# ImIntheMiddle/VATL4Pose-WACV2024

Measured on AMD Instinct MI355X. Metric: frames/sec pose-infer+uncertainty, 256x192 17-kp, higher is better.
Workload: dtype f32; 1 GPU; SimpleBaseline-R50 256x192 inference + decode + local-peak + THC-L1, 1024-frame synthetic video per GPU; frames_per_gpu=1024, batch=1024, tracks=4, parallelism=frame-sharded x1

## Files before the change

### include/vatl_hip.h

```cpp
#ifndef VATL_HIP_H
#define VATL_HIP_H

#include <stdint.h>

#ifdef __cplusplus
extern "C" {
#endif

#define VATL_VERSION 100
#define VATL_EINVAL  (-1)
#define VATL_ELAUNCH (-2)

int         vatl_version(void);
const char* vatl_last_error(void);

int vatl_flop_meter_begin(void);
int vatl_flop_meter_end(double* direct_flops, double* winograd_flops, int64_t* direct_launches, int64_t* winograd_launches);
#define VATL_ROUTE_NAMES "igemm,igemm_bnbwd,igemm_dma,persistent_1x1,streamk,rows_1x1,bottleneck_chain,stem_pool,halo_3x3," \
                         "winograd,winograd_2h,winograd_bnbwd,winograd_persist,winograd_c32,wgrad,winograd_wgrad,winograd_wgrad_2h," \
                         "winograd_wgrad_table,winograd_f4,winograd_f4_bnbwd,gemm1x1_ring"
int vatl_flop_meter_routes(int64_t* counts, int n);


int vatl_nchw_to_nhwc(const float* src, float* dst, int N, int C, int H, int W, int Cpad, void* stream);
int vatl_nhwc_to_nchw(const float* src, float* dst, int N, int C, int H, int W, void* stream);

int vatl_pack_conv_weight(const float* w_oihw, float* w_packed, int Cout, int Cin, int R, int S,
                          int CoutPad, int Spad, int CinPad, void* stream);
int vatl_pack_deconv4x4s2_weight(const float* w_iohw, float* w_packed, int Cin, int Cout, int CoutPad, void* stream);
int64_t vatl_stem_pool_weight_floats(void);
int vatl_pack_stem_pool_weight(const float* w_oihw, float* packed, void* stream);
int vatl_stem_pool_supported(int H, int W);
int vatl_stem7x7s2_pool_fwd(const float* x_nchw, const float* w_packed, const float* scale, const float* bias, float* y_nhwc,
                            int N, int H, int W, void* stream);
int64_t vatl_stem3_weight_floats(void);
int vatl_pack_stem3_weight(const float* w_oihw, float* packed, void* stream);
int vatl_stem3x3s2_fwd(const float* x_nchw, const float* w_packed, const float* scale, const float* bias, float* y_nhwc,
                       int N, int H, int W, void* stream);

int vatl_bn_fold(const float* gamma, const float* beta, const float* mean, const float* var, const float* conv_bias,
                 float eps, float* scale, float* bias, int C, void* stream);


// ... 209 lines not shown
                     int32_t* indices_dev, int32_t* tie_flag_dev, double* workspace, void* stream);
int vatl_kmeans_assign(const double* xc, const double* centers, int64_t n, int D, int k, const int32_t* labels_prev_or_null, int32_t* labels,
                       double* status, double* workspace, void* stream);
int64_t vatl_kmeans_update_workspace_doubles(int D, int k);
int vatl_kmeans_update(const double* xc, const double* weight, const int32_t* labels, const double* centers, int64_t n, int D, int k,
                       double* centers_new, double* status, double* workspace, void* stream);
int vatl_kmeans_finish(const float* emb, const double* xc, const double* mean, const double* weight, const double* centers,
                       const int32_t* labels, int64_t n, int D, int k, int32_t* representatives, double* inertia, double* workspace,
                       void* stream);

int vatl_winograd_cout_pad(int Cout);
int64_t vatl_winograd_weight_floats(int Cout, int Cin);
int vatl_pack_winograd_weight(const float* w, float* u, int Cout, int Cin, int data_gradient, void* stream);
int vatl_conv3x3_winograd_fwd(const float* x, const float* u, const float* scale, const float* bias, const float* residual, float* y,
                              int N, int H, int W, int Cin, int Cout, int relu, void* stream);
int vatl_winograd_last_route(void);
int64_t vatl_winograd_stats_row_blocks(int64_t N, int H, int W);
int vatl_conv3x3_winograd_fwd_stats(const float* x, const float* u, float* y, double* stats, int64_t* row_blocks_used, int N, int H, int W,
                                    int Cin, int Cout, void* stream);
int64_t vatl_winograd_deconv_weight_floats(int Cout, int Cin);
int vatl_pack_winograd_deconv_weight(const float* w, float* u, int Cout, int Cin, void* stream);
int vatl_deconv4x4s2_winograd_fwd(const float* x, const float* u, const float* scale, const float* bias, float* y, int N, int H, int W,
                                  int Cin, int Cout, int relu, void* stream);
int64_t vatl_winograd_deconv_stats_row_blocks(int64_t N, int H, int W);
int vatl_deconv4x4s2_winograd_fwd_stats(const float* x, const float* u, float* y, double* stats, int64_t* row_blocks_used, int N, int H, int W,
                                        int Cin, int Cout, void* stream);
int64_t vatl_conv3x3_winograd_wgrad_workspace_floats(int Cout, int Cin, int64_t N, int H, int W);
int vatl_conv3x3_winograd_wgrad(const float* x, const float* dz, float* dw, float* workspace, int N, int H, int W, int Cin, int Cout, void* stream);
int64_t vatl_deconv4x4s2_winograd_wgrad_workspace_floats(int Cin, int Cout, int64_t N, int H, int W);
int vatl_deconv4x4s2_winograd_wgrad(const float* x, const float* dy, float* dw, float* workspace, int N, int H, int W, int Cin, int Cout,
                                    void* stream);
int64_t vatl_winograd_deconv_dgrad_weight_floats(int Cin, int Cout);
int vatl_pack_winograd_deconv_dgrad_weight(const float* w, float* u, int Cin, int Cout, void* stream);
int vatl_deconv4x4s2_winograd_dgrad(const float* dz, const float* u, const float* residual, float* dx, int N, int H, int W, int Cin, int Cout,
                                    void* stream);
int vatl_deconv4x4s2_winograd_dgrad_bnbwd(const float* dz, const float* u, const float* residual, float* dx, int N, int H, int W, int Cin,
                                          int Cout, const float* bn_z, const float* bn_mask_y, const float* bn_scale, const float* bn_bias,
                                          const float* bn_mean, const float* bn_invstd, double* stats, int64_t* row_blocks_used, void* stream);
int vatl_conv3x3_winograd_fwd_bnbwd(const float* x, const float* u, const float* residual, float* y, int N, int H, int W, int Cin, int Cout,
                                    const float* bn_z, const float* bn_mask_y, const float* bn_scale, const float* bn_bias,
                                    const float* bn_mean, const float* bn_invstd, double* stats, int64_t* row_blocks_used, void* stream);

int64_t vatl_checksum_block_words(void);
int vatl_checksum_multi(const int64_t* table_dev, int n_tensors, int64_t total_blocks, uint64_t* out, void* stream);

#ifdef __cplusplus
// ... 4 lines not shown
```

### vatl4pose-wacv2024_amd/alphapose/models/hip_engine.py

```python
from __future__ import annotations

import time
import weakref

import torch
import torch.nn as nn

import vatl_hip as vh

MAX_CHUNK = 1024



WINOGRAD = True
ROWS_GEMM = True
ROWS_GEMM_K = (128, 256)
WINO_C32 = True
WINO_F4 = True


class _Conv:
    __slots__ = ("w", "u", "u32", "u4", "wsrc", "wino", "c32", "f4", "scale", "bias", "cout", "r", "s", "stride", "pad")

    def __init__(self, conv: nn.Conv2d, bn: nn.BatchNorm2d | None):
        assert conv.groups == 1 and conv.dilation == (1, 1)
        assert conv.stride[0] == conv.stride[1] and conv.padding[0] == conv.padding[1]
        self.w = vh.pack_conv_weight(conv.weight.detach())
        self.cout, _, self.r, self.s = conv.weight.shape
        self.stride, self.pad = conv.stride[0], conv.padding[0]
        self.u = self.u32 = self.u4 = None
        self.wino = WINOGRAD and (self.r, self.s, self.stride, self.pad) == (3, 3, 1, 1) and conv.in_channels % 16 == 0 and self.cout % 4 == 0
        self.c32 = self.wino and WINO_C32 and conv.in_channels == 32 and self.cout == 32
        self.f4 = self.wino and WINO_F4 and conv.in_channels >= 64 and conv.in_channels % 16 == 0 and self.cout % 64 == 0
        self.wsrc = conv.weight.detach() if self.wino else None
        cb = conv.bias.detach() if conv.bias is not None else None
        if bn is not None:
            self.scale, self.bias = vh.bn_fold(_d(bn.weight), _d(bn.bias), bn.running_mean, bn.running_var, bn.eps, cb)
        elif cb is not None:
            self.scale, self.bias = vh.bn_fold(None, None, None, None, 0.0, cb, channels=self.cout)
        else:
            self.scale = self.bias = None

    def __call__(self, x, relu, residual=None, out_nchw=False, out=None):
        if self.wino and not out_nchw and not vh.latency_mode():
            if self.c32 and vh.conv3x3_winograd_c32_supported(x.shape[0], x.shape[1], x.shape[2], 32, 32):
                if self.u32 is None:
                    self.u32 = vh.pack_winograd_c32_weight(self.wsrc)
                return vh.conv3x3_winograd_c32_fwd(x, self.u32, self.scale, self.bias, relu, residual=residual, out=out)
            if self.f4 and vh.conv3x3_winograd_f4_supported(x.shape[0], x.shape[1], x.shape[2], x.shape[3], self.cout):
                if self.u4 is None:
                    self.u4 = vh.pack_winograd_f4_weight(self.wsrc)
                return vh.conv3x3_winograd_f4_fwd(x, self.u4, self.scale, self.bias, self.cout, relu, residual=residual, out=out)
            if self.u is None:
                self.u = vh.pack_winograd_weight(self.wsrc)
            return vh.conv3x3_winograd_fwd(x, self.u, self.scale, self.bias, self.cout, relu, residual=residual, out=out)
        if (ROWS_GEMM and self.r == 1 and self.stride == 1 and not out_nchw and not vh.latency_mode() and x.shape[-1] in ROWS_GEMM_K
                and vh.conv1x1_rows_supported(x.shape[-1], 0, self.cout, x.shape[0] * x.shape[1] * x.shape[2])):
            return vh.conv1x1_rows_fwd(x, self.w, self.scale, self.bias, self.cout, relu, residual=residual, out=out)
        return vh.conv2d_fwd(x, self.w, self.scale, self.bias, self.cout, self.r, self.s, self.stride, self.pad, relu,
                             residual=residual, out_nchw=out_nchw, out=out)


class _Deconv:
    __slots__ = ("w", "u", "scale", "bias", "cout")

    def __init__(self, dc: nn.ConvTranspose2d, bn: nn.BatchNorm2d):
        assert dc.kernel_size == (4, 4) and dc.stride == (2, 2) and dc.padding == (1, 1) and dc.bias is None
        self.cout = dc.weight.shape[1]
        self.u = None
        if WINOGRAD and dc.weight.shape[0] % 16 == 0 and self.cout % 4 == 0:
            self.u = vh.pack_winograd_deconv_weight(dc.weight.detach())
        self.w = vh.pack_deconv_weight(dc.weight.detach())
        self.scale, self.bias = vh.bn_fold(_d(bn.weight), _d(bn.bias), bn.running_mean, bn.running_var, bn.eps)

    def __call__(self, x, relu=True):
        if self.u is not None and not vh.latency_mode():
            return vh.deconv4x4s2_winograd_fwd(x, self.u, self.scale, self.bias, self.cout, relu)
        return vh.deconv4x4s2_fwd(x, self.w, self.scale, self.bias, self.cout, relu)


def _d(p):
    return None if p is None else p.detach()


FUSE_PROJ = True


class _BottleneckPlan:
    def __init__(self, blk):
        self.c1 = _Conv(blk.conv1, blk.bn1)
        self.c2 = _Conv(blk.conv2, blk.bn2)
        self.c3 = _Conv(blk.conv3, blk.bn3)
        self.proj = _Conv(blk.downsample[0], blk.downsample[1]) if blk.downsample is not None else None
        self.dual = None
        if (FUSE_PROJ and self.proj is not None and type(self) is _BottleneckPlan and self.proj.r == 1 and self.c3.cout >= 128
                and blk.conv3.in_channels % 32 == 0 and blk.downsample[0].in_channels % 32 == 0):
            w, b = vh.pack_conv1x1_dual_weight(blk.conv3.weight.detach(), self.c3.scale, self.c3.bias, blk.downsample[0].weight.detach(),
                                               self.proj.scale, self.proj.bias)
            self.dual = (w, b, self.proj.stride)

# ... 469 lines not shown
```

### vatl4pose-wacv2024_amd/csrc/common.h

```cpp
#pragma once
#include <hip/hip_runtime.h>
#include <atomic>
#include <cstdarg>
#include <cstdio>
#include <cstdint>

#include "vatl_hip.h"

namespace vatl {

char* err_buf();
int fail(int code, const char* fmt, ...);

void meter_add(int kind, double flops);
enum MeterRoute {
    kRouteIgemm = 0, kRouteIgemmBnBwd, kRouteIgemmDma, kRoutePersistent1x1, kRouteStreamK, kRouteRows, kRouteChain, kRouteStemPool, kRouteHalo,
    kRouteWino, kRouteWino2H, kRouteWinoBnBwd, kRouteWinoPersist, kRouteWinoC32, kRouteWgrad, kRouteWinoWgrad, kRouteWinoWgrad2H,
    kRouteWinoWgradTable, kRouteWinoF4, kRouteWinoF4BnBwd, kRouteGemm1x1Ring, kRouteCount
};
void meter_route(int route);

inline int check_launch(const char* what) {
    hipError_t e = hipGetLastError();
    if (e != hipSuccess) return fail(VATL_ELAUNCH, "%s: %s", what, hipGetErrorString(e));
    return 0;
}

inline int ensure_dynamic_lds(const void* kern, int bytes, std::atomic<unsigned>& done_mask, const char* what) {
    int d = 0;
    if (hipGetDevice(&d) != hipSuccess) return fail(VATL_ELAUNCH, "%s: no current device", what);
    const unsigned bit = 1u << (d & 31);
    if (done_mask.load(std::memory_order_acquire) & bit) return 0;
    hipError_t e = hipFuncSetAttribute(kern, hipFuncAttributeMaxDynamicSharedMemorySize, bytes);
    if (e != hipSuccess) return fail(VATL_ELAUNCH, "hipFuncSetAttribute(%s): %s", what, hipGetErrorString(e));
    done_mask.fetch_or(bit, std::memory_order_release);
    return 0;
}

__attribute__((visibility("hidden"))) int conv3x3_halo_try(const float* x, const float* w, const float* scale, const float* bias, const float* residual, float* y, int N, int H, int W,
                                                           int Cin, int Cout, int CoutPad, int R, int S, int stride, int pad, int relu, hipStream_t st);

// ... 51 lines not shown
```

### vatl4pose-wacv2024_amd/csrc/pack.hip

```cpp
#include "glue_common.h"
#include "winograd_pack.h"

namespace vatl {

template <class I>
__device__ __forceinline__ float pack_conv_elem(const float* __restrict__ w, I i, int Cout, int Cin, int R, int S, int Spad, int CinPad) {
    const I c = i % (I)CinPad;
    I t = i / (I)CinPad;
    const I s = t % (I)Spad; t /= (I)Spad;
    const I r = t % (I)R;
    const I o = t / (I)R;
    float v = 0.f;
    if ((int)o < Cout && (int)s < S && (int)c < Cin) v = w[(((long long)o * Cin + c) * R + r) * S + s];
    return v;
}

template <class I>
__device__ __forceinline__ float pack_deconv_elem(const float* __restrict__ w, I i, int Cin, int Cout, int CoutPad) {
    const I c = i % (I)Cin;
    I t = i / (I)Cin;
    const int tx = (int)(t & 1); t >>= 1;
    const int ty = (int)(t & 1); t >>= 1;
    const I o = t % (I)CoutPad;
    const int ph = (int)(t / (I)CoutPad);
// ... 54 lines not shown
    for (long long i = blockIdx.x * (long long)blockDim.x + threadIdx.x; i < total; i += (long long)gridDim.x * blockDim.x) {
        const int k = (int)(i % K), o = (int)(i / K);
        float v = 0.f;
        if (o < Cout) v = k < C1 ? w1[(long long)o * C1 + k] * s1[o] : w2[(long long)o * C2 + (k - C1)] * s2[o];
        out[i] = v;
        if (k == 0 && o < Cout) bias[o] = b1[o] + b2[o];
    }
}

__global__ void bn_fold_kernel(const float* gamma, const float* beta, const float* mean, const float* var, const float* cbias,
                               float eps, float* scale, float* bias, int C) {
    const int c = blockIdx.x * blockDim.x + threadIdx.x;
    if (c >= C) return;
    float s = 1.f, b = 0.f;
    if (var) {
        s = (gamma ? gamma[c] : 1.f) / sqrtf(var[c] + eps);
        b = (beta ? beta[c] : 0.f) - mean[c] * s;
    }
    if (cbias) b += cbias[c] * s;
    scale[c] = s;
    bias[c] = b;
}

__global__ __launch_bounds__(256) void pack_multi_kernel(const VatlPackJob* __restrict__ jobs, int njobs) {
    __shared__ int sj;
    if (threadIdx.x == 0) {
        int lo = 0, hi = njobs - 1;
        const long long b = blockIdx.x;
        while (lo < hi) {
            const int mid = (lo + hi + 1) >> 1;
            if (jobs[mid].first_block <= b) lo = mid; else hi = mid - 1;
        }
        sj = lo;
    }
    __syncthreads();
    const VatlPackJob* J = jobs + sj;
    const float* __restrict__ w = J->src;
    float* __restrict__ out = J->dst;
    const int kind = J->kind, Cout = J->Cout, Cin = J->Cin, R = J->R, S = J->S, pa = J->a, pb = J->b, pc = J->c;
    if (kind >= 7) {
        f4_pack_item(w, out, kind - 7, pc, Cout, Cin, ((long long)blockIdx.x - J->first_block) * 256 + threadIdx.x);
        return;
    }
    if (kind >= 3) {
        wino_pack_block(w, out, kind - 3, pc, Cout, Cin, pb, (long long)blockIdx.x - J->first_block, threadIdx.x);
        return;
// ... 20 lines not shown
using namespace vatl;

extern "C" int vatl_pack_conv_weight(const float* w, float* out, int Cout, int Cin, int R, int S, int CoutPad, int Spad, int CinPad, void* stream) {
    if (!w || !out || CoutPad < Cout || Spad < S || CinPad < Cin) return fail(VATL_EINVAL, "pack_conv_weight: bad arguments");
    hipLaunchKernelGGL(pack_conv_weight_kernel, dim3(ew_grid((long long)CoutPad * R * Spad * CinPad)), dim3(256), 0, (hipStream_t)stream,
                       w, out, Cout, Cin, R, S, CoutPad, Spad, CinPad);
    return check_launch("pack_conv_weight");
}

extern "C" int vatl_pack_conv1x1_dual_weight(const float* w1, const float* scale1, const float* bias1, const float* w2, const float* scale2,
                                             const float* bias2, float* out, float* bias, int Cout, int C1, int C2, int CoutPad, void* stream) {
    if (!w1 || !scale1 || !bias1 || !w2 || !scale2 || !bias2 || !out || !bias || CoutPad < Cout) return fail(VATL_EINVAL, "pack_conv1x1_dual_weight: bad arguments");
    hipLaunchKernelGGL(pack_dual_weight_kernel, dim3(ew_grid((long long)CoutPad * (C1 + C2))), dim3(256), 0, (hipStream_t)stream, w1, scale1, bias1, w2,
                       scale2, bias2, out, bias, Cout, C1, C2, CoutPad);
    return check_launch("pack_conv1x1_dual_weight");
}

extern "C" int vatl_pack_deconv4x4s2_weight(const float* w, float* out, int Cin, int Cout, int CoutPad, void* stream) {
    if (!w || !out || CoutPad < Cout) return fail(VATL_EINVAL, "pack_deconv4x4s2_weight: bad arguments");
    hipLaunchKernelGGL(pack_deconv_weight_kernel, dim3(ew_grid(16LL * CoutPad * Cin)), dim3(256), 0, (hipStream_t)stream, w, out, Cin, Cout, CoutPad);
    return check_launch("pack_deconv4x4s2_weight");
}

extern "C" int vatl_pack_dgrad_weight(const float* w_oihw, float* out, int Cout, int Cin, int R, int S, int CinPad, int CoutK,
                                      int ntaps, const int* tap_r, const int* tap_s, void* stream) {
    if (!w_oihw || !out || !tap_r || !tap_s || ntaps < 1 || ntaps > 16 || CinPad < Cin || CoutK < Cout) return fail(VATL_EINVAL, "pack_dgrad_weight: bad arguments");
    TapList t{};
    t.n = ntaps;
    for (int i = 0; i < ntaps; ++i) {
        if (tap_r[i] < 0 || tap_r[i] >= R || tap_s[i] < 0 || tap_s[i] >= S) return fail(VATL_EINVAL, "pack_dgrad_weight: tap %d out of range", i);
        t.r[i] = tap_r[i]; t.s[i] = tap_s[i];
    }
    hipLaunchKernelGGL(pack_dgrad_weight_kernel, dim3((unsigned)((long long)cdiv(CinPad, 32) * ntaps * cdiv(CoutK, 32))), dim3(256), 0, (hipStream_t)stream,
                       w_oihw, out, Cout, Cin, R, S, CinPad, CoutK, t);
    return check_launch("pack_dgrad_weight");
}

extern "C" int vatl_pack_weights_multi(const VatlPackJob* jobs_device, int njobs, int64_t total_blocks, void* stream) {
    if (njobs == 0) return 0;
    if (!jobs_device || njobs < 0 || total_blocks <= 0 || total_blocks > 0x7FFFFFFF) return fail(VATL_EINVAL, "pack_weights_multi: bad arguments");
    hipLaunchKernelGGL(pack_multi_kernel, dim3((unsigned)total_blocks), dim3(256), 0, (hipStream_t)stream, jobs_device, njobs);
    return check_launch("pack_weights_multi");
}

extern "C" int vatl_bn_fold(const float* gamma, const float* beta, const float* mean, const float* var, const float* conv_bias,
                            float eps, float* scale, float* bias, int C, void* stream) {
// ... 5 lines not shown
```

### vatl4pose-wacv2024_amd/csrc/winograd_pack.h

```cpp
#pragma once

namespace vatl {

__device__ __forceinline__ void wino_pack_block(const float* __restrict__ w, float* __restrict__ out, int mode, int w_i, int Cout, int Cin, int NH,
                                                long long bl, int tid) {
    const int steps = Cin >> 3;
    int phase = 0;
    if (mode >= 2) {
        const long long per = (long long)((Cout + 32 * NH - 1) / (32 * NH)) * NH * steps;
        phase = (int)(bl / per);
        bl -= phase * per;
        out += phase * per * 4096;
    }
    const int n32 = (int)(bl / steps), step = (int)(bl - (long long)n32 * steps);
    const int nl = tid & 31, cc = tid >> 5;
    const int n = n32 * 32 + nl, c = step * 8 + cc;
    const int n_tile = n32 / NH, nh = n32 - n_tile * NH;
    const int lane = (cc >> 2) * 32 + nl, tt = cc & 3;
    double tg[4][3];
    if (mode >= 2) {
        const int py = phase >> 1, px = phase & 1;
        double g[2][2];
#pragma unroll
        for (int a = 0; a < 2; ++a)
// ... 20 lines not shown
                double v = 0.0;
                if (n < Cout) v = mode == 0 ? (double)w[((long long)n * w_i + c) * 9 + r * 3 + s] : (double)w[((long long)c * w_i + n) * 9 + (2 - r) * 3 + (2 - s)];
                g[r][s] = v;
            }
#pragma unroll
        for (int s = 0; s < 3; ++s) {
            tg[0][s] = g[0][s];
            tg[1][s] = 0.5 * (g[0][s] + g[1][s] + g[2][s]);
            tg[2][s] = 0.5 * (g[0][s] - g[1][s] + g[2][s]);
            tg[3][s] = g[2][s];
        }
    }
    float* o = out + ((((long long)(n_tile * steps + step) * 16) * NH + nh) * 64 + lane) * 4 + tt;
#pragma unroll
    for (int a = 0; a < 4; ++a) {
        double uu[4];
        if (mode >= 2) { uu[0] = tg[a][0]; uu[1] = 0.5 * (tg[a][0] + tg[a][1]); uu[2] = 0.5 * (tg[a][0] - tg[a][1]); uu[3] = -tg[a][1]; }
        else { uu[0] = tg[a][0]; uu[1] = 0.5 * (tg[a][0] + tg[a][1] + tg[a][2]); uu[2] = 0.5 * (tg[a][0] - tg[a][1] + tg[a][2]); uu[3] = tg[a][2]; }
#pragma unroll
        for (int b = 0; b < 4; ++b) o[(long long)(a * 4 + b) * NH * 256] = (float)uu[b];
    }
}

__device__ __forceinline__ void f4_pack_item(const float* __restrict__ w, float* __restrict__ u, int dgrad, int w_i, int Cout, int Cin, long long id) {
    const int nbg = Cout >> 4;
    const long long total = (long long)(Cin >> 4) * 36 * nbg * 64;
    if (id >= total) return;
    const int lane = (int)(id & 63);
    const int blk = (int)((id >> 6) % nbg);
    const int pos = (int)((id >> 6) / nbg % 36);
    const int stage = (int)((id >> 6) / nbg / 36);
    const int xi = pos / 6, nu = pos - 6 * xi;
    const double G[6][3] = {{0.25, 0, 0}, {-1.0 / 6, -1.0 / 6, -1.0 / 6}, {-1.0 / 6, 1.0 / 6, -1.0 / 6}, {1.0 / 24, 1.0 / 12, 1.0 / 6}, {1.0 / 24, -1.0 / 12, 1.0 / 6}, {0, 0, 1}};
    const int n = 16 * blk + (lane & 15);
    float o[4];
#pragma unroll
    for (int s = 0; s < 4; ++s) {
        const int c = 16 * stage + 4 * (lane >> 4) + s;
        const float* g = dgrad ? w + ((long long)c * w_i + n) * 9 : w + ((long long)n * w_i + c) * 9;
        double v = 0.0;
#pragma unroll
        for (int i = 0; i < 3; ++i)
#pragma unroll
            for (int j = 0; j < 3; ++j) v += G[xi][i] * (double)(dgrad ? g[(2 - i) * 3 + (2 - j)] : g[i * 3 + j]) * G[nu][j];
        o[s] = (float)v;
    }
// ... 6 lines not shown
```

### vatl4pose-wacv2024_amd/vatl_hip/__init__.py

```python
from __future__ import annotations

import ctypes as C
import os
import threading as _threading

import torch

_HERE = os.path.dirname(os.path.abspath(__file__))
LIB_PATH = os.environ.get("VATL_HIP_LIB") or os.path.join(_HERE, "libvatl_hip.so")

_p = C.c_void_p
_i = C.c_int
_f = C.c_float
_d = C.c_double
_i64 = C.c_int64

SIGNATURES = {
    "vatl_version": (_i, []),
    "vatl_last_error": (C.c_char_p, []),
    "vatl_flop_meter_begin": (_i, []),
    "vatl_flop_meter_end": (_i, [_p, _p, _p, _p]),
    "vatl_flop_meter_routes": (_i, [_p, _i]),
    "vatl_nchw_to_nhwc": (_i, [_p, _p, _i, _i, _i, _i, _i, _p]),
    "vatl_nhwc_to_nchw": (_i, [_p, _p, _i, _i, _i, _i, _p]),
# ... 65 lines not shown
    "vatl_scale_bias_act": (_i, [_p, _p, _p, _p, _p, _i64, _i, _i, _p]),
    "vatl_bn_train_bwd": (_i, [_p, _p, _p, _p, _p, _p, _p, _p, _p, _p, _i64, _i, _p, _p, _p]),
    "vatl_bn_train_bwd_relu": (_i, [_p, _p, _p, _p, _p, _p, _p, _p, _p, _p, _i64, _i, _p, _p, _p]),
    "vatl_conv_stats_row_blocks": (_i64, [_i64, _i]),
    "vatl_winograd_cout_pad": (_i, [_i]),
    "vatl_winograd_weight_floats": (_i64, [_i, _i]),
    "vatl_pack_winograd_weight": (_i, [_p, _p, _i, _i, _i, _p]),
    "vatl_conv3x3_winograd_fwd": (_i, [_p] * 6 + [_i] * 6 + [_p]),
    "vatl_winograd_last_route": (_i, []),
    "vatl_winograd_stats_row_blocks": (_i64, [_i64, _i, _i]),
    "vatl_conv3x3_winograd_fwd_stats": (_i, [_p, _p, _p, _p, _p, _i, _i, _i, _i, _i, _p]),
    "vatl_conv3x3_winograd_fwd_bnbwd": (_i, [_p] * 4 + [_i] * 5 + [_p] * 9),
    "vatl_conv3x3_winograd_wgrad_workspace_floats": (_i64, [_i, _i, _i64, _i, _i]),
    "vatl_conv3x3_winograd_wgrad": (_i, [_p] * 4 + [_i] * 5 + [_p]),
    "vatl_deconv4x4s2_winograd_wgrad_workspace_floats": (_i64, [_i, _i, _i64, _i, _i]),
    "vatl_deconv4x4s2_winograd_wgrad": (_i, [_p] * 4 + [_i] * 5 + [_p]),
    "vatl_winograd_deconv_dgrad_weight_floats": (_i64, [_i, _i]),
    "vatl_pack_winograd_deconv_dgrad_weight": (_i, [_p, _p, _i, _i, _p]),
    "vatl_deconv4x4s2_winograd_dgrad": (_i, [_p] * 4 + [_i] * 5 + [_p]),
    "vatl_deconv4x4s2_winograd_dgrad_bnbwd": (_i, [_p] * 4 + [_i] * 5 + [_p] * 9),
    "vatl_winograd_deconv_weight_floats": (_i64, [_i, _i]),
    "vatl_pack_winograd_deconv_weight": (_i, [_p, _p, _i, _i, _p]),
    "vatl_deconv4x4s2_winograd_fwd": (_i, [_p] * 5 + [_i] * 6 + [_p]),
    "vatl_winograd_deconv_stats_row_blocks": (_i64, [_i64, _i, _i]),
    "vatl_deconv4x4s2_winograd_fwd_stats": (_i, [_p, _p, _p, _p, _p, _i, _i, _i, _i, _i, _p]),
    "vatl_conv2d_fwd_stats": (_i, [_p, _p, _p, _p, _p, _i, _i, _i, _i, _i, _i, _i, _i, _i, _i, _p]),
    "vatl_deconv4x4s2_fwd_stats": (_i, [_p, _p, _p, _p, _p, _i, _i, _i, _i, _i, _i, _p]),
    "vatl_bn_train_finalize": (_i, [_p, _i64, _i64, _i, _p, _p, _p, _p, _f, _f, _p, _p, _p, _p, _p]),
    "vatl_maxpool3x3s2_bwd": (_i, [_p, _p, _p, _i, _i, _i, _i, _p]),
    "vatl_maxpool3x3s2_fwd_idx": (_i, [_p, _p, _p, _i, _i, _i, _i, _p]),
    "vatl_pack_weights_multi": (_i, [_p, _i, _i64, _p]),
    "vatl_adamw_multi_block_elems": (_i64, []),
    "vatl_checksum_block_words": (_i64, []),
    "vatl_checksum_multi": (_i, [_p, _i, _i64, _p, _p]),
    "vatl_maxpool3x3s2_fwd_idx_affine": (_i, [_p, _p, _p, _p, _p, _i, _i, _i, _i, _p]),
    "vatl_bn_train_bwd_relu_pool": (_i, [_p, _p, _p, _p, _p, _p, _p, _p, _p, _p, _p, _i, _i, _i, _i, _p, _p, _p]),
    "vatl_maxpool3x3s2_bwd_idx": (_i, [_p, _p, _p, _i, _i, _i, _i, _p]),
    "vatl_pixelunshuffle2": (_i, [_p, _p, _i, _i, _i, _i, _p]),
    "vatl_se_bwd": (_i, [_p, _p, _p, _p, _p, _p, _p, _p, _i, _i, _i, _p]),
    "vatl_relu_bwd": (_i, [_p, _p, _p, _i64, _p]),
    "vatl_col_sum": (_i, [_p, _i64, _i, _p, _p, _p]),
    "vatl_masked_mse_workspace_floats": (_i64, [_i64]),
    "vatl_masked_mse_fwd_bwd": (_i, [_p, _p, _p, _p, _p, _p, _i, _i, _i, _p]),
    "vatl_l1_joint_regression_fwd_bwd": (_i, [_p, _p, _p, _p, _p, _p, _p, _i, _i, _i, _i, _i, _i, _p]),
    "vatl_gaussian_targets": (_i, [_p, _p, _p, _p, _i, _i, _i, _i, _i, _i, _f, _p]),
    "vatl_crop_warp_affine": (_i, [_p, _p, _p, _p, _p, _p, _i, _i, _i, _f, _f, _f, _p]),
# ... 82 lines not shown

_tls = _threading.local()



def nchw_to_nhwc(x: torch.Tensor, cpad: int | None = None) -> torch.Tensor:
    n, c, h, w = x.shape
    cpad = cpad or c
    y = torch.empty((n, h, w, cpad), device=x.device, dtype=torch.float32)
    _check(lib().vatl_nchw_to_nhwc(_ptr(x), _ptr(y), n, c, h, w, cpad, _stream()), "vatl_nchw_to_nhwc")
    return y


def nhwc_to_nchw(x: torch.Tensor) -> torch.Tensor:
    n, h, w, c = x.shape
    y = torch.empty((n, c, h, w), device=x.device, dtype=torch.float32)
    _check(lib().vatl_nhwc_to_nchw(_ptr(x), _ptr(y), n, c, h, w, _stream()), "vatl_nhwc_to_nchw")
    return y



ROUTE_NAMES = ("igemm", "igemm_bnbwd", "igemm_dma", "persistent_1x1", "streamk", "rows_1x1", "bottleneck_chain", "stem_pool", "halo_3x3", "winograd",
               "winograd_2h", "winograd_bnbwd", "winograd_persist", "winograd_c32", "wgrad", "winograd_wgrad", "winograd_wgrad_2h", "winograd_wgrad_table", "winograd_f4", "winograd_f4_bnbwd",
               "gemm1x1_ring")


class flop_meter:

    def __enter__(self):
        _check(lib().vatl_flop_meter_begin(), "flop_meter_begin")
        self.direct = self.winograd = self.total = 0.0
        self.direct_launches = self.winograd_launches = 0
        return self

    @staticmethod
    def launches_now() -> int:
        counts = (C.c_int64 * len(ROUTE_NAMES))()
        _check(min(0, lib().vatl_flop_meter_routes(counts, len(ROUTE_NAMES))), "flop_meter_routes")
        return int(sum(counts))

    def __exit__(self, *exc):
        counts = (C.c_int64 * len(ROUTE_NAMES))()
        _check(min(0, lib().vatl_flop_meter_routes(counts, len(ROUTE_NAMES))), "flop_meter_routes")
        self.routes = {n: int(c) for n, c in zip(ROUTE_NAMES, counts)}
        d, w, nd, nw = C.c_double(0), C.c_double(0), C.c_int64(0), C.c_int64(0)
        _check(lib().vatl_flop_meter_end(C.byref(d), C.byref(w), C.byref(nd), C.byref(nw)), "flop_meter_end")
        self.direct, self.winograd, self.total = d.value, w.value, d.value + w.value
# ... 240 lines not shown
    cout, cin = (ci, co) if data_gradient else (co, ci)
    return _pack(("winograd", w.data_ptr(), tuple(w.shape), bool(data_gradient)), w, lambda: (
        int(lib().vatl_winograd_weight_floats(cout, cin)), "vatl_pack_winograd_weight", (cout, cin, int(data_gradient)),
        _winograd_fields(_PACK_WINOGRAD_DGRAD if data_gradient else _PACK_WINOGRAD, cout, cin, 3, ci)))


def pack_winograd_f4_weight(w: torch.Tensor, data_gradient: bool = False) -> torch.Tensor:
    co, ci = w.shape[:2]
    cout, cin = (ci, co) if data_gradient else (co, ci)
    return _pack(("winograd_f4", w.data_ptr(), tuple(w.shape), bool(data_gradient)), w, lambda: (
        int(lib().vatl_winograd_f4_weight_floats(cout, cin)), "vatl_pack_winograd_f4_weight", (cout, cin, int(data_gradient)),
        (_PACK_WINOGRAD_F4_DGRAD if data_gradient else _PACK_WINOGRAD_F4, cout, cin, 3, 3, 0, 0, ci, ())))


def pack_winograd_deconv_weight(w: torch.Tensor) -> torch.Tensor:
    cin, cout = w.shape[:2]
    if tuple(w.shape[2:]) != (4, 4):
        raise VatlError("pack_winograd_deconv_weight: 4x4 filters only")
    return _pack(("winograd_deconv", w.data_ptr(), tuple(w.shape)), w, lambda: (
        int(lib().vatl_winograd_deconv_weight_floats(cout, cin)), "vatl_pack_winograd_deconv_weight", (cout, cin),
        _winograd_fields(_PACK_WINOGRAD_DECONV, cout, cin, 4, cout)))


def pack_winograd_deconv_dgrad_weight(w: torch.Tensor) -> torch.Tensor:
    cin, cout = w.shape[:2]
    if tuple(w.shape[2:]) != (4, 4):
        raise VatlError("pack_winograd_deconv_dgrad_weight: 4x4 filters only")
    return _pack(("winograd_deconv_dgrad", w.data_ptr(), tuple(w.shape)), w, lambda: (
        int(lib().vatl_winograd_deconv_dgrad_weight_floats(cin, cout)), "vatl_pack_winograd_deconv_dgrad_weight", (cin, cout),
        _winograd_fields(_PACK_WINOGRAD_DECONV_DGRAD, cin, cout, 4, cout)))


def pack_conv1x1_dual_weight(w1, scale1, bias1, w2, scale2, bias2):
    cout, c1 = w1.shape[:2]
    c2 = w2.shape[1]
    cpad = conv_cout_pad(cout)
    out = torch.empty((cpad, c1 + c2), device=w1.device, dtype=torch.float32)
    bias = torch.empty(cout, device=w1.device, dtype=torch.float32)
    _check(lib().vatl_pack_conv1x1_dual_weight(_ptr(w1.contiguous()), _ptr(scale1), _ptr(bias1), _ptr(w2.contiguous()), _ptr(scale2), _ptr(bias2),
                                               _ptr(out), _ptr(bias), cout, c1, c2, cpad, _stream()), "vatl_pack_conv1x1_dual_weight")
    return out, bias


def pack_winograd_c32_weight(w: torch.Tensor) -> torch.Tensor:
    if tuple(w.shape) != (32, 32, 3, 3):
        raise VatlError("pack_winograd_c32_weight: a (32, 32, 3, 3) filter")
# ... 126 lines not shown
    return y


def conv3x3_winograd_f4_supported(n: int, h: int, w: int, cin: int, cout: int) -> bool:
    return bool(lib().vatl_conv3x3_winograd_f4_supported(n, h, w, cin, cout))


def conv3x3_winograd_f4_fwd(x, u, scale, bias, cout: int, relu: bool, residual=None, out=None):
    n, h, w, cin = x.shape
    y = out if out is not None else torch.empty((n, h, w, cout), device=x.device, dtype=torch.float32)
    _check(lib().vatl_conv3x3_winograd_f4_fwd(_ptr(x), _ptr(u), _ptr(scale), _ptr(bias), _ptr(residual), _ptr(y), n, h, w, cin, cout, int(relu), _stream()),
           "vatl_conv3x3_winograd_f4_fwd")
    return y


def deconv4x4s2_fwd(x, w_packed, scale, bias, cout: int, relu: bool):
    n, h, w, cin = x.shape
    y = torch.empty((n, 2 * h, 2 * w, cout), device=x.device, dtype=torch.float32)
    _check(lib().vatl_deconv4x4s2_fwd(_ptr(x), _ptr(w_packed), _ptr(scale), _ptr(bias), _ptr(y), n, h, w, cin, cout,
                                      w_packed.shape[1], int(relu), _stream()), "vatl_deconv4x4s2_fwd")
    return y


def deconv4x4s2_winograd_fwd(x, u_packed, scale, bias, cout: int, relu: bool, out=None):
    n, h, w, cin = x.shape
    y = out if out is not None else torch.empty((n, 2 * h, 2 * w, cout), device=x.device, dtype=torch.float32)
    _check(lib().vatl_deconv4x4s2_winograd_fwd(_ptr(x), _ptr(u_packed), _ptr(scale), _ptr(bias), _ptr(y), n, h, w, cin, cout, int(relu), _stream()),
           "vatl_deconv4x4s2_winograd_fwd")
    return y


def maxpool3x3s2_fwd(x):
    n, h, w, c = x.shape
    y = torch.empty((n, (h - 1) // 2 + 1, (w - 1) // 2 + 1, c), device=x.device, dtype=torch.float32)
    _check(lib().vatl_maxpool3x3s2_fwd(_ptr(x), _ptr(y), n, h, w, c, _stream()), "vatl_maxpool3x3s2_fwd")
    return y


def gap_fwd(x):
    n, h, w, c = x.shape
    y = torch.empty((n, c), device=x.device, dtype=torch.float32)
    _check(lib().vatl_gap_fwd(_ptr(x), _ptr(y), n, h * w, c, _stream()), "vatl_gap_fwd")
    return y


def pixelshuffle2_fwd(x):
    n, h, w, c = x.shape
    y = torch.empty((n, 2 * h, 2 * w, c // 4), device=x.device, dtype=torch.float32)
    _check(lib().vatl_pixelshuffle2_fwd(_ptr(x), _ptr(y), n, h, w, c, _stream()), "vatl_pixelshuffle2_fwd")
# ... 751 lines not shown
```

Before: 16340 frames/s.

## Add F(4x3,2x2) Winograd kernel for stride-2 deconvolution phases

Adds a new Winograd kernel for the 4x4 stride-2 deconvolution. Each of the four output phases is treated as a 2x2 conv and computed with larger output tiles: 4 rows by 3 columns and 20 transform points. The kernel uses MFMA 32x32x2 f32, buffer loads straight into LDS, double-buffered stages and XCD-aware block remapping. The aim is fewer multiplies per output and better reuse than the existing deconv Winograd path. The packed weights are built lazily on the first supported call. The trade-offs are extra numerical error from the larger transform, an extra packed-weight buffer, and shape restrictions (H%4, W%3, Cout%64).

```diff
diff --git a/include/vatl_hip.h b/include/vatl_hip.h
--- a/include/vatl_hip.h
+++ b/include/vatl_hip.h
@@ -18,7 +18,7 @@
 int vatl_flop_meter_end(double* direct_flops, double* winograd_flops, int64_t* direct_launches, int64_t* winograd_launches);
 #define VATL_ROUTE_NAMES "igemm,igemm_bnbwd,igemm_dma,persistent_1x1,streamk,rows_1x1,bottleneck_chain,stem_pool,halo_3x3," \
                          "winograd,winograd_2h,winograd_bnbwd,winograd_persist,winograd_c32,wgrad,winograd_wgrad,winograd_wgrad_2h," \
-                         "winograd_wgrad_table,winograd_f4,winograd_f4_bnbwd,gemm1x1_ring"
+                         "winograd_wgrad_table,winograd_f4,winograd_f4_bnbwd,gemm1x1_ring,winograd_deconv43"
 int vatl_flop_meter_routes(int64_t* counts, int n);
 
 
@@ -274,6 +274,11 @@
 int vatl_pack_winograd_deconv_weight(const float* w, float* u, int Cout, int Cin, void* stream);
 int vatl_deconv4x4s2_winograd_fwd(const float* x, const float* u, const float* scale, const float* bias, float* y, int N, int H, int W,
                                   int Cin, int Cout, int relu, void* stream);
+int64_t vatl_winograd_deconv43_weight_floats(int Cout, int Cin);
+int vatl_pack_winograd_deconv43_weight(const float* w, float* u, int Cout, int Cin, void* stream);
+int vatl_deconv4x4s2_winograd43_supported(int N, int H, int W, int Cin, int Cout);
+int vatl_deconv4x4s2_winograd43_fwd(const float* x, const float* u, const float* scale, const float* bias, float* y, int N, int H, int W,
+                                    int Cin, int Cout, int relu, void* stream);
 int64_t vatl_winograd_deconv_stats_row_blocks(int64_t N, int H, int W);
 int vatl_deconv4x4s2_winograd_fwd_stats(const float* x, const float* u, float* y, double* stats, int64_t* row_blocks_used, int N, int H, int W,
                                         int Cin, int Cout, void* stream);
diff --git a/vatl4pose-wacv2024_amd/alphapose/models/hip_engine.py b/vatl4pose-wacv2024_amd/alphapose/models/hip_engine.py
--- a/vatl4pose-wacv2024_amd/alphapose/models/hip_engine.py
+++ b/vatl4pose-wacv2024_amd/alphapose/models/hip_engine.py
@@ -17,6 +17,7 @@
 ROWS_GEMM_K = (128, 256)
 WINO_C32 = True
 WINO_F4 = True
+DECONV_43 = True
 
 
 class _Conv:
@@ -62,12 +63,14 @@
 
 
 class _Deconv:
-    __slots__ = ("w", "u", "scale", "bias", "cout")
+    __slots__ = ("w", "u", "u43", "wsrc", "d43", "scale", "bias", "cout")
 
     def __init__(self, dc: nn.ConvTranspose2d, bn: nn.BatchNorm2d):
         assert dc.kernel_size == (4, 4) and dc.stride == (2, 2) and dc.padding == (1, 1) and dc.bias is None
         self.cout = dc.weight.shape[1]
-        self.u = None
+        self.u = self.u43 = None
+        self.d43 = WINOGRAD and DECONV_43 and dc.weight.shape[0] % 16 == 0 and self.cout % 64 == 0
+        self.wsrc = dc.weight.detach() if self.d43 else None
         if WINOGRAD and dc.weight.shape[0] % 16 == 0 and self.cout % 4 == 0:
             self.u = vh.pack_winograd_deconv_weight(dc.weight.detach())
         self.w = vh.pack_deconv_weight(dc.weight.detach())
@@ -75,7 +78,9 @@
 
     def __call__(self, x, relu=True):
         if self.u is not None and not vh.latency_mode():
-            return vh.deconv4x4s2_winograd_fwd(x, self.u, self.scale, self.bias, self.cout, relu)
+            if self.d43 and self.u43 is None and vh.deconv4x4s2_winograd43_supported(x.shape[0], x.shape[1], x.shape[2], x.shape[3], self.cout):
+                self.u43 = vh.pack_winograd_deconv43_weight(self.wsrc)
+            return vh.deconv4x4s2_winograd_fwd(x, self.u, self.scale, self.bias, self.cout, relu, u43=self.u43)
         return vh.deconv4x4s2_fwd(x, self.w, self.scale, self.bias, self.cout, relu)
 
 
diff --git a/vatl4pose-wacv2024_amd/csrc/common.h b/vatl4pose-wacv2024_amd/csrc/common.h
--- a/vatl4pose-wacv2024_amd/csrc/common.h
+++ b/vatl4pose-wacv2024_amd/csrc/common.h
@@ -16,7 +16,7 @@
 enum MeterRoute {
     kRouteIgemm = 0, kRouteIgemmBnBwd, kRouteIgemmDma, kRoutePersistent1x1, kRouteStreamK, kRouteRows, kRouteChain, kRouteStemPool, kRouteHalo,
     kRouteWino, kRouteWino2H, kRouteWinoBnBwd, kRouteWinoPersist, kRouteWinoC32, kRouteWgrad, kRouteWinoWgrad, kRouteWinoWgrad2H,
-    kRouteWinoWgradTable, kRouteWinoF4, kRouteWinoF4BnBwd, kRouteGemm1x1Ring, kRouteCount
+    kRouteWinoWgradTable, kRouteWinoF4, kRouteWinoF4BnBwd, kRouteGemm1x1Ring, kRouteWinoDeconv43, kRouteCount
 };
 void meter_route(int route);
 
diff --git a/vatl4pose-wacv2024_amd/csrc/pack.hip b/vatl4pose-wacv2024_amd/csrc/pack.hip
--- a/vatl4pose-wacv2024_amd/csrc/pack.hip
+++ b/vatl4pose-wacv2024_amd/csrc/pack.hip
@@ -100,6 +100,10 @@
     bias[c] = b;
 }
 
+__global__ __launch_bounds__(256) void wino43_pack_kernel(const float* __restrict__ w, float* __restrict__ out, int Cout, int Cin) {
+    wino43_pack_block(w, out, Cout, Cin, blockIdx.x, threadIdx.x);
+}
+
 __global__ __launch_bounds__(256) void pack_multi_kernel(const VatlPackJob* __restrict__ jobs, int njobs) {
     __shared__ int sj;
     if (threadIdx.x == 0) {
@@ -166,6 +170,17 @@
     return check_launch("pack_deconv4x4s2_weight");
 }
 
+extern "C" int64_t vatl_winograd_deconv43_weight_floats(int Cout, int Cin) { return 4LL * 20 * Cout * Cin; }
+
+extern "C" int vatl_pack_winograd_deconv43_weight(const float* w, float* u, int Cout, int Cin, void* stream) {
+    if (!w || !u || Cout <= 0 || Cin <= 0) return fail(VATL_EINVAL, "pack_winograd_deconv43_weight: null pointer or empty filter");
+    if (Cin % 16 != 0 || Cout % 64 != 0) return fail(VATL_EINVAL, "pack_winograd_deconv43_weight: Cin %d must be a multiple of 16 and Cout %d of 64", Cin, Cout);
+    const long long blocks = 4LL * (Cout / 32) * (Cin / 8);
+    if (blocks > 0x7FFFFFFF) return fail(VATL_EINVAL, "pack_winograd_deconv43_weight: filter too large");
+    hipLaunchKernelGGL(wino43_pack_kernel, dim3((unsigned)blocks), dim3(256), 0, (hipStream_t)stream, w, u, Cout, Cin);
+    return check_launch("wino43_pack");
+}
+
 extern "C" int vatl_pack_dgrad_weight(const float* w_oihw, float* out, int Cout, int Cin, int R, int S, int CinPad, int CoutK,
                                       int ntaps, const int* tap_r, const int* tap_s, void* stream) {
     if (!w_oihw || !out || !tap_r || !tap_s || ntaps < 1 || ntaps > 16 || CinPad < Cin || CoutK < Cout) return fail(VATL_EINVAL, "pack_dgrad_weight: bad arguments");
diff --git a/vatl4pose-wacv2024_amd/csrc/winograd_deconv43.hip b/vatl4pose-wacv2024_amd/csrc/winograd_deconv43.hip
--- /dev/null
+++ b/vatl4pose-wacv2024_amd/csrc/winograd_deconv43.hip
@@ -0,0 +1,292 @@
+#include "common.h"
+#include "buffer.h"
+#include "winograd_pack.h"
+
+#include <algorithm>
+#include <atomic>
+
+namespace vatl {
+
+struct Deconv43Params {
+    const float* x;
+    const float* u;
+    const float* scale;
+    const float* bias;
+    float* y;
+    int N, H, W, Cin, Cout;
+    int TH, TW, tpi, Mtiles;
+    int m_tiles, n_tiles;
+    int relu;
+    int stages;
+    int rn;
+    long long u_phase_floats;
+    unsigned x_bytes, u_bytes, y_bytes;
+    FastDivU d_TH, d_TW, d_tpi, d_grp, d_rn, d_rn_last, d_ntiles;
+};
+
+constexpr unsigned D43_OOB = 0xFFFF0000u;
+constexpr int D43_TB = 32;
+constexpr int D43_CK = 16;
+constexpr int D43_NQ = D43_TB + 1;
+constexpr int D43_ROWE = 3 * D43_NQ + 1;
+constexpr int D43_ROWF = D43_ROWE * D43_CK;
+constexpr int D43_ITEMS = 5 * D43_ROWE * 4;
+constexpr int D43_NDMA = (D43_ITEMS + 63) / 64;
+constexpr int D43_STAGE = D43_NDMA * 256;
+constexpr int D43_NLD = D43_NDMA / 4;
+constexpr int D43_LDS_BYTES = 2 * D43_STAGE * 4;
+static_assert(D43_NDMA % 4 == 0 && 16 * D43_TB * 32 * 4 == D43_LDS_BYTES, "stage buffers = output-transform tiles");
+
+__device__ __forceinline__ void winograd_deconv43_body(const Deconv43Params& p, float* smem) {
+    constexpr int NW = 4;
+    float* Rs = smem;
+    const int tid = threadIdx.x, lane = tid & 63, nu = __builtin_amdgcn_readfirstlane(tid >> 6);
+
+    const int bid = blockIdx.x, nblk = gridDim.x;
+    const int xcd = bid & 7, loc = bid >> 3, q8 = nblk >> 3, r8 = nblk & 7;
+    const int t = (xcd < r8 ? xcd * (q8 + 1) : r8 * (q8 + 1) + (xcd - r8) * q8) + loc;
+    const int units = p.n_tiles * 4;
+    const int grp = fdiv(t, p.d_grp), rem = t - grp * (p.m_tiles * p.rn);
+    const bool last_grp = units - grp * p.rn < p.rn;
+    const int rn_g = last_grp ? units - grp * p.rn : p.rn;
+    const int m_tile = fdiv(rem, last_grp ? p.d_rn_last : p.d_rn), unit = grp * p.rn + (rem - m_tile * rn_g);
+    const int phase = fdiv(unit, p.d_ntiles), n_tile = unit - phase * p.n_tiles;
+    const int m0 = m_tile * D43_TB, n0 = n_tile * 64;
+    const int py = phase >> 1, px = phase & 1;
+    const int pad_y = 1 - py, pad_x = 1 - px;
+
+    const __amdgpu_buffer_rsrc_t xr = buf_rsrc(p.x, p.x_bytes);
+    const __amdgpu_buffer_rsrc_t ur = buf_rsrc(p.u + (long long)phase * p.u_phase_floats, p.u_bytes);
+
+    const int steps = p.stages * 2;
+    const unsigned ubase = (unsigned)(((n_tile * steps) * 20 + nu) * 2 * 64 + lane) << 4;
+    auto u_load = [&](f32x4 (&dst)[5], int step_, int half) {
+        const int step = min(step_, steps - 1);
+        const unsigned off = ubase + (unsigned)half * 1024u + (unsigned)step * 40960u;
+#pragma unroll
+        for (int xi = 0; xi < 5; ++xi) dst[xi] = buf_load4(ur, off + xi * 8192u);
+    };
+    f32x4 ua[5], ub[5];
+    u_load(ua, 0, 0);
+
+    unsigned goff[D43_NLD];
+#pragma unroll
+    for (int u = 0; u < D43_NLD; ++u) {
+        const int pz = (nu + NW * u) * 64 + lane;
+        goff[u] = D43_OOB;
+        if (pz >= D43_ITEMS) continue;
+        const int cpos = pz & 3, e = pz >> 2;
+        const int i = e / D43_ROWE, re = e - i * D43_ROWE;
+        const int r = re / D43_NQ, q = re - r * D43_NQ;
+        if (r >= 3) continue;
+        const int chunk = cpos ^ ((q >> 2) & 3);
+        int m = m0 + q;
+        int gr = fdiv(m, p.d_TW), tx = m - gr * p.TW;
+        int xx = 3 * tx + r - pad_x;
+        if (m >= p.Mtiles || (tx == 0 && xx < 0)) {
+            m -= 1;
+            if (m < 0) continue;
+            gr = fdiv(m, p.d_TW); tx = m - gr * p.TW;
+            xx = 3 * tx + 3 + r - pad_x;
+        }
+        const int b = fdiv(gr, p.d_TH), ty = gr - b * p.TH;
+        const int yy = 4 * ty - pad_y + i;
+        if (m < p.Mtiles && (unsigned)yy < (unsigned)p.H && (unsigned)xx < (unsigned)p.W)
+            goff[u] = (unsigned)(((b * p.H + yy) * p.W + xx) * p.Cin + chunk * 4) << 2;
+    }
+    auto stage_dma = [&](int buf, int st) {
+#pragma unroll
+        for (int u = 0; u < D43_NLD; ++u)
+            __builtin_amdgcn_raw_ptr_buffer_load_lds(xr, (lds_void*)(Rs + buf * D43_STAGE + (nu + NW * u) * 256), 16,
+                                                     goff[u] + (unsigned)st * (D43_CK * 4), 0, 0, 0);
+    };
+    stage_dma(0, 0);
+    if (p.stages > 1) stage_dma(1, 1);
+
+    const int h = lane >> 5;
+    const int ja = nu == 0 ? 0 : (nu == 2 ? 2 : 1);
+    const int jb = nu == 0 ? 2 : (nu == 1 ? 2 : (nu == 2 ? 1 : 3));
+    const float sgn = nu == 1 ? 1.f : -1.f;
+    int ca, cb;
+    {
+        const int tl = lane & 31;
+        const int m = min(m0 + tl, p.Mtiles - 1);
+        const int gr = fdiv(m, p.d_TW), tx = m - gr * p.TW;
+        auto col = [&](int j) {
+            const int xx = 3 * tx + j - pad_x;
+            const int q = tl + j / 3;
+            return (unsigned)xx < (unsigned)p.W ? ((j % 3) * D43_NQ + q) * D43_CK + ((h ^ ((q >> 2) & 3)) << 2) : 3 * D43_NQ * D43_CK + (h << 2);
+        };
+        ca = col(ja); cb = col(jb);
+    }
+
+    f32x16 accs[2][5];
+#pragma unroll
+    for (int hh = 0; hh < 2; ++hh)
+#pragma unroll
+        for (int xi = 0; xi < 5; ++xi)
+#pragma unroll
+            for (int e = 0; e < 16; ++e) accs[hh][xi][e] = 0.f;
+
+    asm volatile("s_waitcnt vmcnt(0)" ::: "memory");
+    __syncthreads();
+
+    auto make_v = [&](f32x4 (&v)[5], const float* Rb, int x8) {
+        f32x4 tc[5];
+#pragma unroll
+        for (int i = 0; i < 5; ++i) {
+            const f32x4 da = *reinterpret_cast<const f32x4*>(Rb + i * D43_ROWF + (ca ^ x8));
+            const f32x4 db = *reinterpret_cast<const f32x4*>(Rb + i * D43_ROWF + (cb ^ x8));
+            tc[i] = da + sgn * db;
+        }
+        const f32x4 s = tc[3] - tc[1];
+        v[0] = 2.f * (tc[0] - tc[2]) + s;
+        v[1] = s - (tc[1] + tc[2]);
+        v[2] = 2.f * tc[1] + (tc[3] - 3.f * tc[2]);
+        v[3] = s;
+        v[4] = (tc[4] - tc[2]) - 2.f * s;
+    };
+    auto mfma_group = [&](f32x16 (&ac)[5], const f32x4 (&v)[5], const f32x4 (&uu)[5]) {
+#pragma unroll
+        for (int tt = 0; tt < 4; ++tt)
+#pragma unroll
+            for (int xi = 0; xi < 5; ++xi)
+                ac[xi] = __builtin_amdgcn_mfma_f32_32x32x2f32(v[xi][tt], uu[xi][tt], ac[xi], 0, 0, 0);
+    };
+
+    for (int st = 0; st < p.stages; ++st) {
+        const int buf = st & 1;
+        const float* Rb = Rs + buf * D43_STAGE;
+        f32x4 v[5];
+        u_load(ub, 2 * st, 1);
+        __builtin_amdgcn_sched_barrier(0);
+        make_v(v, Rb, 0);
+        mfma_group(accs[0], v, ua);
+        __builtin_amdgcn_sched_barrier(0);
+        u_load(ua, 2 * st + 1, 0);
+        __builtin_amdgcn_sched_barrier(0);
+        mfma_group(accs[1], v, ub);
+        __builtin_amdgcn_sched_barrier(0);
+        u_load(ub, 2 * st + 1, 1);
+        if (st + 1 < p.stages && st > 0) stage_dma(buf ^ 1, st + 1);
+        __builtin_amdgcn_sched_barrier(0);
+        make_v(v, Rb, 8);
+        mfma_group(accs[0], v, ua);
+        __builtin_amdgcn_sched_barrier(0);
+        u_load(ua, 2 * st + 2, 0);
+        __builtin_amdgcn_sched_barrier(0);
+        mfma_group(accs[1], v, ub);
+        __builtin_amdgcn_sched_barrier(0);
+        asm volatile("s_waitcnt vmcnt(0)" ::: "memory");
+        __syncthreads();
+    }
+
+    const __amdgpu_buffer_rsrc_t yr = buf_rsrc(p.y, p.y_bytes);
+    const int c4 = tid & 7, tl = tid >> 3;
+    const int OW = 2 * p.W;
+    const unsigned cstep = (unsigned)(2 * p.Cout) << 2, rstep = (unsigned)(2 * OW * p.Cout) << 2;
+    const bool valid = m0 + tl < p.Mtiles;
+    unsigned obase;
+    {
+        const int m = min(m0 + tl, p.Mtiles - 1);
+        const int b = fdiv(m, p.d_tpi), r = m - b * p.tpi;
+        const int ty = fdiv(r, p.d_TW), tx = r - ty * p.TW;
+        obase = (unsigned)(((b * 2 * p.H + 8 * ty + py) * OW + 6 * tx + px) * p.Cout + n0 + c4 * 4) << 2;
+    }
+    const float lo = p.relu ? 0.f : -INFINITY;
+    float* Ps = smem;
+#pragma unroll
+    for (int hh = 0; hh < 2; ++hh) {
+        const int n = n0 + 32 * hh + c4 * 4;
+        f32x4 sc = {1.f, 1.f, 1.f, 1.f}, bi = {0.f, 0.f, 0.f, 0.f};
+        if (p.scale) sc = *reinterpret_cast<const f32x4*>(p.scale + n);
+        if (p.bias) bi = *reinterpret_cast<const f32x4*>(p.bias + n);
+        {
+            const int cl = lane & 31;
+            f32x16 (&ac)[5] = accs[hh];
+#pragma unroll
+            for (int e = 0; e < 16; ++e) {
+                const int row = (e & 3) + 8 * (e >> 2) + 4 * (lane >> 5);
+                const float sum = ac[1][e] + ac[2][e], dif = ac[1][e] - ac[2][e], m3 = ac[3][e];
+                Ps[((nu * 4 + 0) * D43_TB + row) * 32 + cl] = ac[0][e] + sum + m3;
+                Ps[((nu * 4 + 1) * D43_TB + row) * 32 + cl] = dif + 2.f * m3;
+                Ps[((nu * 4 + 2) * D43_TB + row) * 32 + cl] = sum + 4.f * m3;
+                Ps[((nu * 4 + 3) * D43_TB + row) * 32 + cl] = dif + 8.f * m3 + ac[4][e];
+            }
+        }
+        lds_barrier();
+#pragma unroll
+        for (int a = 0; a < 4; ++a) {
+            f32x4 pq[4];
+#pragma unroll
+            for (int k = 0; k < 4; ++k) pq[k] = *reinterpret_cast<const f32x4*>(&Ps[((k * 4 + a) * D43_TB + tl) * 32 + c4 * 4]);
+            f32x4 yv[3];
+            yv[0] = pq[0] + pq[1] + pq[2];
+            yv[1] = pq[1] - pq[2];
+            yv[2] = pq[1] + pq[2] + pq[3];
+            if (valid) {
+#pragma unroll
+                for (int b = 0; b < 3; ++b) {
+                    f32x4 o;
+#pragma unroll
+                    for (int c = 0; c < 4; ++c) o[c] = fmaxf(yv[b][c] * sc[c] + bi[c], lo);
+                    buf_store4(yr, obase + (unsigned)hh * 128u + (unsigned)a * rstep + (unsigned)b * cstep, o);
+                }
+            }
+        }
+        if (hh == 0) lds_barrier();
+    }
+}
+
+__global__ __launch_bounds__(256, 2) void winograd_deconv43_kernel(Deconv43Params p) {
+    extern __shared__ __attribute__((aligned(16))) float smem[];
+    winograd_deconv43_body(p, smem);
+}
+
+static std::atomic<unsigned> g_d43_lds_done;
+
+static bool d43_in_range(long long N, int H, int W, int Cin, int Cout) {
+    const long long mt = N * (H / 4) * (W / 3), xe = N * H * W * Cin, ye = 4 * N * H * W * Cout, ue = 20LL * Cout * Cin;
+    return xe <= (long long)(D43_OOB / 4) && ye < (1LL << 30) && ue < (1LL << 28) && mt < (1LL << 30) && Cin / D43_CK < 1024 &&
+           (mt + D43_TB - 1) / D43_TB * (Cout / 64) * 4 < (1LL << 31);
+}
+
+}
+
+using namespace vatl;
+
+extern "C" int vatl_deconv4x4s2_winograd43_supported(int N, int H, int W, int Cin, int Cout) {
+    if (N <= 0 || H <= 0 || W <= 0 || Cin <= 0 || Cout <= 0) return 0;
+    if (H % 4 != 0 || W % 3 != 0 || Cin % 16 != 0 || Cout % 64 != 0) return 0;
+    return d43_in_range(N, H, W, Cin, Cout) ? 1 : 0;
+}
+
+extern "C" int vatl_deconv4x4s2_winograd43_fwd(const float* x, const float* u, const float* scale, const float* bias, float* y, int N, int H, int W,
+                                               int Cin, int Cout, int relu, void* stream) {
+    if (!x || !u || !y) return fail(VATL_EINVAL, "deconv4x4s2_winograd43_fwd: null pointer");
+    if (!vatl_deconv4x4s2_winograd43_supported(N, H, W, Cin, Cout))
+        return fail(VATL_EINVAL, "deconv4x4s2_winograd43_fwd: %d x %dx%d x %d -> %d is outside H %% 4 == 0, W %% 3 == 0, Cin %% 16 == 0, Cout %% 64 == 0 and 32-bit offsets",
+                    N, H, W, Cin, Cout);
+    Deconv43Params p{};
+    p.x = x; p.u = u; p.scale = scale; p.bias = bias; p.y = y;
+    p.N = N; p.H = H; p.W = W; p.Cin = Cin; p.Cout = Cout; p.relu = relu;
+    p.TH = H / 4; p.TW = W / 3; p.tpi = p.TH * p.TW;
+    p.Mtiles = N * p.tpi;
+    p.m_tiles = cdiv(p.Mtiles, D43_TB);
+    p.n_tiles = Cout / 64;
+    p.stages = Cin / D43_CK;
+    p.u_phase_floats = 20LL * Cout * Cin;
+    p.x_bytes = (unsigned)((long long)N * H * W * Cin * 4);
+    p.y_bytes = (unsigned)(4LL * N * H * W * Cout * 4);
+    p.u_bytes = (unsigned)(p.u_phase_floats * 4);
+    const int units = p.n_tiles * 4;
+    p.rn = std::max(1, std::min(units, std::max(2, 2048 / (5 * Cin))));
+    p.d_TH = make_fastdiv(p.TH); p.d_TW = make_fastdiv(p.TW); p.d_tpi = make_fastdiv(p.tpi);
+    p.d_grp = make_fastdiv((unsigned)(p.m_tiles * p.rn)); p.d_rn = make_fastdiv(p.rn); p.d_ntiles = make_fastdiv(p.n_tiles);
+    p.d_rn_last = make_fastdiv(units % p.rn ? units % p.rn : p.rn);
+    if (int rc = ensure_dynamic_lds((const void*)winograd_deconv43_kernel, D43_LDS_BYTES, g_d43_lds_done, "winograd_deconv43")) return rc;
+    hipLaunchKernelGGL(winograd_deconv43_kernel, dim3((unsigned)(p.m_tiles * units)), dim3(256), D43_LDS_BYTES, (hipStream_t)stream, p);
+    meter_add(1, 2.0 * ((double)p.m_tiles * D43_TB) * 20.0 * (double)Cin * (double)Cout * 4.0);
+    meter_route(kRouteWinoDeconv43);
+    return check_launch("winograd_deconv43");
+}
diff --git a/vatl4pose-wacv2024_amd/csrc/winograd_pack.h b/vatl4pose-wacv2024_amd/csrc/winograd_pack.h
--- a/vatl4pose-wacv2024_amd/csrc/winograd_pack.h
+++ b/vatl4pose-wacv2024_amd/csrc/winograd_pack.h
@@ -66,6 +66,37 @@
     }
 }
 
+__device__ __forceinline__ void wino43_pack_block(const float* __restrict__ w, float* __restrict__ out, int Cout, int Cin, long long bl, int tid) {
+    const int steps = Cin >> 3;
+    const long long per = (long long)(Cout >> 5) * steps;
+    const int phase = (int)(bl / per);
+    bl -= phase * per;
+    out += phase * per * 5120;
+    const int n32 = (int)(bl / steps), step = (int)(bl - (long long)n32 * steps);
+    const int nl = tid & 31, cc = tid >> 5;
+    const int n = n32 * 32 + nl, c = step * 8 + cc;
+    const int py = phase >> 1, px = phase & 1;
+    const double G4[5][2] = {{0.5, 0.0}, {-0.5, -0.5}, {-1.0 / 6, 1.0 / 6}, {1.0 / 6, 1.0 / 3}, {0.0, 1.0}};
+    const double G3[4][2] = {{1.0, 0.0}, {0.5, 0.5}, {0.5, -0.5}, {0.0, -1.0}};
+    double g[2][2];
+#pragma unroll
+    for (int a = 0; a < 2; ++a)
+#pragma unroll
+        for (int b = 0; b < 2; ++b) g[a][b] = (double)w[(((long long)c * Cout + n) * 4 + (3 - py - 2 * a)) * 4 + (3 - px - 2 * b)];
+    float* o = out + ((((long long)((n32 >> 1) * steps + step) * 20) * 2 + (n32 & 1)) * 64 + (cc >> 2) * 32 + nl) * 4 + (cc & 3);
+#pragma unroll
+    for (int xi = 0; xi < 5; ++xi)
+#pragma unroll
+        for (int nu = 0; nu < 4; ++nu) {
+            double v = 0.0;
+#pragma unroll
+            for (int a = 0; a < 2; ++a)
+#pragma unroll
+                for (int b = 0; b < 2; ++b) v += G4[xi][a] * g[a][b] * G3[nu][b];
+            o[(long long)(xi * 4 + nu) * 512] = (float)v;
+        }
+}
+
 __device__ __forceinline__ void f4_pack_item(const float* __restrict__ w, float* __restrict__ u, int dgrad, int w_i, int Cout, int Cin, long long id) {
     const int nbg = Cout >> 4;
     const long long total = (long long)(Cin >> 4) * 36 * nbg * 64;
diff --git a/vatl4pose-wacv2024_amd/vatl_hip/__init__.py b/vatl4pose-wacv2024_amd/vatl_hip/__init__.py
--- a/vatl4pose-wacv2024_amd/vatl_hip/__init__.py
+++ b/vatl4pose-wacv2024_amd/vatl_hip/__init__.py
@@ -111,6 +111,10 @@
     "vatl_winograd_deconv_weight_floats": (_i64, [_i, _i]),
     "vatl_pack_winograd_deconv_weight": (_i, [_p, _p, _i, _i, _p]),
     "vatl_deconv4x4s2_winograd_fwd": (_i, [_p] * 5 + [_i] * 6 + [_p]),
+    "vatl_winograd_deconv43_weight_floats": (_i64, [_i, _i]),
+    "vatl_pack_winograd_deconv43_weight": (_i, [_p, _p, _i, _i, _p]),
+    "vatl_deconv4x4s2_winograd43_supported": (_i, [_i, _i, _i, _i, _i]),
+    "vatl_deconv4x4s2_winograd43_fwd": (_i, [_p] * 5 + [_i] * 6 + [_p]),
     "vatl_winograd_deconv_stats_row_blocks": (_i64, [_i64, _i, _i]),
     "vatl_deconv4x4s2_winograd_fwd_stats": (_i, [_p, _p, _p, _p, _p, _i, _i, _i, _i, _i, _p]),
     "vatl_conv2d_fwd_stats": (_i, [_p, _p, _p, _p, _p, _i, _i, _i, _i, _i, _i, _i, _i, _i, _i, _p]),
@@ -239,7 +243,7 @@
 
 ROUTE_NAMES = ("igemm", "igemm_bnbwd", "igemm_dma", "persistent_1x1", "streamk", "rows_1x1", "bottleneck_chain", "stem_pool", "halo_3x3", "winograd",
                "winograd_2h", "winograd_bnbwd", "winograd_persist", "winograd_c32", "wgrad", "winograd_wgrad", "winograd_wgrad_2h", "winograd_wgrad_table", "winograd_f4", "winograd_f4_bnbwd",
-               "gemm1x1_ring")
+               "gemm1x1_ring", "winograd_deconv43")
 
 
 class flop_meter:
@@ -526,6 +530,14 @@
         _winograd_fields(_PACK_WINOGRAD_DECONV, cout, cin, 4, cout)))
 
 
+def pack_winograd_deconv43_weight(w: torch.Tensor) -> torch.Tensor:
+    cin, cout = w.shape[:2]
+    if tuple(w.shape[2:]) != (4, 4):
+        raise VatlError("pack_winograd_deconv43_weight: 4x4 filters only")
+    return _pack(("winograd_deconv43", w.data_ptr(), tuple(w.shape)), w, lambda: (
+        int(lib().vatl_winograd_deconv43_weight_floats(cout, cin)), "vatl_pack_winograd_deconv43_weight", (cout, cin), None), planned=False)
+
+
 def pack_winograd_deconv_dgrad_weight(w: torch.Tensor) -> torch.Tensor:
     cin, cout = w.shape[:2]
     if tuple(w.shape[2:]) != (4, 4):
@@ -698,9 +710,17 @@
     return y
 
 
-def deconv4x4s2_winograd_fwd(x, u_packed, scale, bias, cout: int, relu: bool, out=None):
+def deconv4x4s2_winograd43_supported(n: int, h: int, w: int, cin: int, cout: int) -> bool:
+    return bool(lib().vatl_deconv4x4s2_winograd43_supported(n, h, w, cin, cout))
+
+
+def deconv4x4s2_winograd_fwd(x, u_packed, scale, bias, cout: int, relu: bool, out=None, u43=None):
     n, h, w, cin = x.shape
     y = out if out is not None else torch.empty((n, 2 * h, 2 * w, cout), device=x.device, dtype=torch.float32)
+    if u43 is not None and deconv4x4s2_winograd43_supported(n, h, w, cin, cout):
+        _check(lib().vatl_deconv4x4s2_winograd43_fwd(_ptr(x), _ptr(u43), _ptr(scale), _ptr(bias), _ptr(y), n, h, w, cin, cout, int(relu), _stream()),
+               "vatl_deconv4x4s2_winograd43_fwd")
+        return y
     _check(lib().vatl_deconv4x4s2_winograd_fwd(_ptr(x), _ptr(u_packed), _ptr(scale), _ptr(bias), _ptr(y), n, h, w, cin, cout, int(relu), _stream()),
            "vatl_deconv4x4s2_winograd_fwd")
     return y
```

New measurement: 16680 frames/s (median of 6 runs). 2.1% higher.
